# XiangLi2022/CM-TTS

Measured on AMD Instinct MI355X. Metric: mel-frames/s (text->mel hot path, consistency sampling T=4), higher is better.
Workload: dtype f32

## Files before the change

cm-tts_amd/csrc/denoiser_persist.hip:

```cpp
#include <hip/hip_runtime.h>
#include <type_traits>
#include "gate.h"
#include "mfma_lane.h"
#include "persist_args.h"
#include "persist_tail.h"
#include "wino43.h"

typedef float f32x2 __attribute__((ext_vector_type(2)));

#ifndef WINO_ABL
#define WINO_ABL 0
#endif
#ifndef WINO_L2PF
#define WINO_L2PF 0
#endif
#ifndef WINO_THREAD
#define WINO_THREAD 1
#endif
#ifndef WINO43_RING
#define WINO43_RING 3
#endif
#ifndef WINO_RING
#define WINO_RING 3
#endif

namespace {

constexpr int C = 256;
constexpr int NW = 8;
constexpr int MT = 2;
constexpr int RING = 6;
constexpr int FN = 64;
constexpr int NT = FN / 32;
constexpr int U_LD = FN + 4;
constexpr int ROWV = 4 * 32;
constexpr int IDX_LDS_BYTES = (FN + 2) * 2 * 4 + NW * 64 * 4 + NW * 4 + NW * ROWV * 4;
static_assert(((FN + 2) * 2 * 4 + NW * 64 * 4 + NW * 4) % 16 == 0, "row vectors are read 16 bytes at a time");
constexpr unsigned SPIN_LIMIT = 1u << 20;


template <bool DBG, bool RAGGED, bool FACT = false, int WINO = 0>
__global__ __launch_bounds__(64 * NW, 2) void denoiser_persist_kernel(const PersistArgs a) {
    extern __shared__ __attribute__((aligned(16))) float smem[];
    const int tid = threadIdx.x, lane = tid & 63, w = tid >> 6;
    int tile_, b_, T_, Tc_, gi = 0;
    if (RAGGED) {
        const unsigned d = a.desc[blockIdx.x];
        gi = d & 7;
        b_ = (d >> 3) & 1023;
        tile_ = (d >> 13) & 127;
        T_ = a.grp[gi].T;
        Tc_ = min(T_, (int)((d >> 20) & 255) * FN);
    } else {
        tile_ = blockIdx.x; b_ = blockIdx.y; T_ = a.T; Tc_ = a.T;
    }
    const int tile = tile_, b = b_;
    const int t0 = tile * FN;
    const int T = T_;
    const int Tc = Tc_;
    const int l31 = lane & 31, khalf = lane >> 5;
    const float* x0_b = (RAGGED ? a.grp[gi].x0 : a.x0) + (long)b * C * T;
    const float* cp_b = (RAGGED ? a.grp[gi].cp + (long)b * a.grp[gi].cp_bstride : a.cp + (long)b * a.cp_bstride);
    const float* dp_b = (RAGGED ? a.grp[gi].dp : a.dp) + (long)b * a.vec_stride;
    const float* dv_b = (RAGGED ? a.grp[gi].d : a.d) + (long)b * a.vec_stride;
    unsigned long long* halo_g = RAGGED ? a.grp[gi].halo : a.halo;
    const int B_g = RAGGED ? a.grp[gi].B : a.B, tiles_g = RAGGED ? a.grp[gi].tiles : a.tiles;
    const int mrow0 = w * 32;
    const float *p1_b = nullptr, *p1t_b = nullptr;
    const long long *m2p_b = nullptr, *pix_b = nullptr;
    int ldp = 0, Lph = 0;
    if (FACT) {
        p1_b = (RAGGED ? a.grp[gi].p1 : a.p1);
        ldp = RAGGED ? a.grp[gi].ldp : a.ldp;
        Lph = RAGGED ? a.grp[gi].Lph : a.Lph;
        p1_b += (long)b * a.NL * C * ldp;
        p1t_b = (RAGGED ? a.grp[gi].p1t : a.p1t) + (long)b * a.NL * C * ldp;
        m2p_b = (RAGGED ? a.grp[gi].mel2ph : a.mel2ph) + (long)b * T;
        pix_b = (RAGGED ? a.grp[gi].pidx : a.pidx) + (long)b * T;
    }
    auto frame_idx = [&](int t_c, int& ph, int& ix) {
        const long long p = m2p_b[t_c], q = pix_b[t_c];
        ph = (int)(p > Lph ? Lph : p);
        ix = q < 0 ? 0 : (q >= a.ld2 ? a.ld2 - 1 : (int)q);
    };
    auto cp_fact = [&](int row, int ph, int ix) -> float {
        const float av = p1_b[(long)row * ldp + (ph > 0 ? ph - 1 : 0)];
        const float qv = a.p2[(long)row * a.ld2 + ix];
        return (ph > 0 ? av : 0.f) + qv;
    };

    auto uidx = [](int f) { return WINO == 1 ? ((f & 1) ? (f + 1) >> 1 : 33 + (f >> 1)) : f + 1; };
    constexpr int PST_TILE = NW * 8 * 64 * 4;
    float* pst_b = nullptr;
    if (WINO) pst_b = (RAGGED ? a.grp[gi].xst : a.xst) + ((long)b * (RAGGED ? a.grp[gi].tiles : a.tiles) + tile) * PST_TILE;

    {
        const float* xin = x0_b;
        const int t = t0 + lane;
        const int t_c = min(t, T - 1);
        int ph0 = 0, ix0 = 0;
        if (FACT) frame_idx(t_c, ph0, ix0);
        constexpr int ROWS_PER_WAVE = C / NW;
#pragma unroll 1
        for (int i = 0; i < ROWS_PER_WAVE; i += 8) {
            float xv[8], cv[8], dq[8];
#pragma unroll
            for (int q = 0; q < 8; ++q) {
                const int m = w * ROWS_PER_WAVE + i + q;
                xv[q] = xin[(unsigned)(m * T + t_c)];
                cv[q] = FACT ? cp_fact(m, ph0, ix0) : cp_b[(unsigned)(m * T + t_c)];
                dq[q] = dp_b[m];
            }
#pragma unroll
            for (int q = 0; q < 8; ++q) {
                const int m = w * ROWS_PER_WAVE + i + q;
                const float uv = cv[q] + (xv[q] + dq[q]);
                smem[m * U_LD + uidx(lane)] = t < Tc ? uv : 0.f;
            }
        }
        if (tid < 2 * C) {
            const int m = tid & (C - 1);
            const bool right = tid >= C;
            const int th = right ? t0 + FN : t0 - 1;
            const int thc = min(max(th, 0), T - 1);
            float cph0;
            if (FACT) { int ph, ix; frame_idx(thc, ph, ix); cph0 = cp_fact(m, ph, ix); }
            else cph0 = cp_b[(unsigned)(m * T + thc)];
            const float uh = cph0 + (xin[(unsigned)(m * T + thc)] + dp_b[m]);
            smem[m * U_LD + uidx(right ? FN : -1)] = (th >= 0 && th < Tc) ? uh : 0.f;
        }
    }
    int* idx_lds = reinterpret_cast<int*>(smem + 2 * C * U_LD);
    int* zflag = idx_lds + (FN + 2) * 2 + NW * 64;
    if (tid < NW) zflag[tid] = 0;
    float* rowv = reinterpret_cast<float*>(zflag + NW) + w * ROWV;
    constexpr bool ROWV_LDS = WINO != 0;
    if (FACT && tid < FN + 2) {
        int ph, ix;
        frame_idx(min(max(t0 - 1 + tid, 0), T - 1), ph, ix);
        idx_lds[2 * tid] = ph;
        idx_lds[2 * tid + 1] = ix;
    }
    f32x16 st[MT][NT];
    {
        const float* xin = x0_b;
#pragma unroll
        for (int i = 0; i < MT; ++i)
#pragma unroll
            for (int j = 0; j < NT; ++j) {
                const int t_c = min(t0 + j * 32 + l31, T - 1);
#pragma unroll
                for (int r = 0; r < 16; ++r)
                    st[i][j][r] = (i == 0 && !WINO) ? ldg(xin, (unsigned)((mrow0 + acc_row(r, lane)) * T + t_c)) : 0.f;
            }
    }

    f32x16 acc[MT][NT];
    auto load_a = [&](f32x4 (&dst)[MT], const float* wfrag, int group) {
#pragma unroll
        for (int i = 0; i < MT; ++i)
            dst[i] = *reinterpret_cast<const f32x4*>(wfrag + ((long)group * (2 * C / 32) + w * MT + i) * 256 + lane * 4);
    };
    auto load_ao = [&](f32x4 (&dst)[MT], const float* wfrag, int group) {
#pragma unroll
        for (int i = 0; i < MT; ++i)
            dst[i] = *reinterpret_cast<const f32x4*>(wfrag + ((long)group * (2 * C / 32) + i * NW + w) * 256 + lane * 4);
    };
    const f32x16 zero16 = {0.f, 0.f, 0.f, 0.f, 0.f, 0.f, 0.f, 0.f, 0.f, 0.f, 0.f, 0.f, 0.f, 0.f, 0.f, 0.f};
    auto mma_group = [&](auto first, const f32x4 (&af)[MT], const float (&bv)[4][NT], auto i0) {
        constexpr bool FIRST = decltype(first)::value;
        constexpr int I0 = decltype(i0)::value;
#pragma unroll
        for (int kk = 0; kk < 4; ++kk)
#pragma unroll
            for (int i = I0; i < MT; ++i)
#pragma unroll
                for (int j = 0; j < NT; ++j)
                    acc[i][j] = __builtin_amdgcn_mfma_f32_32x32x2f32(af[i][kk], bv[kk][j], FIRST && kk == 0 ? zero16 : acc[i][j], 0, 0, 0);
    };
    using first_t = std::integral_constant<bool, true>;
    using later_t = std::integral_constant<bool, false>;

    const int bid_dbg = blockIdx.x + gridDim.x * blockIdx.y;
#ifdef PUB_STAMP
    constexpr bool PUBS = true;
#else
    constexpr bool PUBS = false;
#endif
    constexpr int DBG_SLOTS = 9;
    auto stamp = [&](int l, int slot) {
        if (DBG && a.dbg && lane == 0) {
            long long* d = a.dbg + ((long)bid_dbg * NW + w) * DBG_SLOTS;
            if (l == a.NL / 2 && !(PUBS && slot < 6)) d[slot] = (long long)__builtin_readcyclecounter();
            if (l == a.NL / 2 + 1 && slot == 0) d[8] = (long long)__builtin_readcyclecounter();
        }
    };
    auto pstamp = [&](int l, int slot) {
        if (DBG && PUBS && a.dbg && l == a.NL / 2 && lane == 0) {
            asm volatile("s_waitcnt lgkmcnt(0)" ::: "memory");
            a.dbg[((long)bid_dbg * NW + w) * DBG_SLOTS + slot] = (long long)__builtin_readcyclecounter();
        }
    };
    bool gave_up = false;
    for (int l = 0; l < a.NL; ++l) {
        float* u_lds = smem;
        float* z_lds = smem + C * U_LD;
        const bool more = l + 1 < a.NL;
        constexpr int NGB = (C / 8) * 3;
        constexpr int NGC = C / 8;
        auto kgrp = [&](int it, int& g8, int& tap) {
            it = min(it, NGB - 1);
            const int q = it / 6, rr = it - q * 6;
            tap = rr >> 1;
            g8 = 2 * q + (rr & 1);
        };
        f32x4 A[RING][MT];
        constexpr int WR = WINO_RING, NH = C / 4;
        f32x4 Aw[WINO == 1 ? WR : 1][MT][2];
        constexpr int WR4 = WINO43_RING, NS4 = C / 4;
        f32x4 A4[WINO == 2 ? WR4 : 1][6];
        auto load_a4 = [&](f32x4 (&dst)[6], const float* wfrag, int ks) {
            const __amdgpu_buffer_rsrc_t rs = __builtin_amdgcn_make_buffer_rsrc(const_cast<float*>(wfrag), 0, (NS4 + 4) * (NW * 6 * 64 * 16), 0x00020000);
            const int voff = (w * 6 * 64 + lane) * 16;
#pragma unroll
            for (int p = 0; p < 6; ++p)
                dst[p] = __builtin_bit_cast(f32x4, __builtin_amdgcn_raw_buffer_load_b128(rs, voff + p * 1024, ks * (NW * 6 * 64 * 16), 0));
        };
        auto load_aw = [&](f32x4 (&dst)[MT][2], const float* wfrag, int hg) {
            const char* base = reinterpret_cast<const char*>(wfrag) + (size_t)hg * ((2 * C / 32) * 2 * 64 * 16);
#pragma unroll
            for (int i = 0; i < MT; ++i)
#pragma unroll
                for (int ps = 0; ps < 2; ++ps)
                    dst[i][ps] = *reinterpret_cast<const f32x4*>(base + (size_t)((unsigned)((((w * MT + i) * 2 + ps) * 64 + lane) * 16)));
        };
        if (WINO == 2) {
#pragma unroll
            for (int s = 0; s < WR4 - 1; ++s) load_a4(A4[s], a.W3f[l], s);
        } else if (WINO == 1) {
#pragma unroll
            for (int s = 0; s < WR - 1; ++s) load_aw(Aw[s], a.W3f[l], s);
        } else {
            int g8, tap;
#pragma unroll
            for (int s = 0; s < RING - 1; ++s) {
                kgrp(s, g8, tap);
                load_a(A[s], a.W3f[l], tap * (C / 8) + g8);
            }
        }
        stamp(l, 0);
        __syncthreads();
        stamp(l, 1);
        if (!FACT && more && tid < 2 * C) {
            const float* cpn = cp_b + (long)(l + 1) * C * T;
            const int tl = opaque(tid);
            const float warm = cpn[(unsigned)((tl >> 1) * T + min(t0 + (tl & 1) * 32, T - 1))];
            asm volatile("" ::"v"(warm));
        }

        f32x16 accw[WINO == 1 ? MT : 1][WINO == 1 ? 4 : 1];
        f32x4 acc4[WINO == 2 ? 4 : 1][WINO == 2 ? 6 : 1];
        if constexpr (WINO == 2) {
#pragma unroll
            for (int i = 0; i < 4; ++i)
#pragma unroll
                for (int p = 0; p < 6; ++p)
#pragma unroll
                    for (int r = 0; r < 4; ++r) acc4[i][p][r] = 0.f;
            const float* W3f = a.W3f[l];
            float V4[6];
            f32x4 Da;
            float2 Db;
            auto load_d4 = [&](int ks) {
                const float* rr = u_lds + (4 * ks + (lane >> 4)) * U_LD + 4 * (lane & 15);
                Da = *reinterpret_cast<const f32x4*>(rr);
                Db = *reinterpret_cast<const float2*>(rr + 4);
            };
            auto transform4 = [&]() { wino43::transform(Da, Db, V4); };
            load_d4(0);
#pragma unroll 1
            for (int s0 = 0; s0 < NS4; s0 += WR4) {
#pragma unroll
                for (int s = 0; s < WR4; ++s) {
                    const int ks = s0 + s;
                    transform4();
                    __builtin_amdgcn_sched_barrier(0);
                    load_a4(A4[(s + WR4 - 1) % WR4], W3f, ks + WR4 - 1);
                    load_d4(ks + 1);
                    if (ks < NS4) {
#pragma unroll
                        for (int p = 0; p < 6; ++p)
#pragma unroll
                            for (int i = 0; i < 4; ++i)
                                acc4[i][p] = __builtin_amdgcn_mfma_f32_16x16x4f32(A4[s][p][i], V4[p], acc4[i][p], 0, 0, 0);
                    }
                    __builtin_amdgcn_sched_barrier(0);
                }
            }
        } else if constexpr (WINO == 1) {
#pragma unroll
            for (int i = 0; i < MT; ++i)
#pragma unroll
                for (int tr = 0; tr < 4; ++tr)
#pragma unroll
                    for (int r = 0; r < 16; ++r) accw[i][tr][r] = 0.f;
            const float* W3f = a.W3f[l];
            float Vb[2][4], Dn[2][4];
            auto load_d = [&](int hg) {
                const float* bs = u_lds + (4 * hg + khalf) * U_LD + l31;
#pragma unroll
                for (int kk = 0; kk < 2; ++kk) {
                    const float* rr = bs + 2 * kk * U_LD;
                    Dn[kk][0] = rr[0]; Dn[kk][2] = rr[1]; Dn[kk][1] = rr[33]; Dn[kk][3] = rr[34];
                }
            };
            auto transform = [&]() {
#pragma unroll
                for (int kk = 0; kk < 2; ++kk) {
                    Vb[kk][0] = Dn[kk][0] - Dn[kk][2];
                    Vb[kk][1] = Dn[kk][1] + Dn[kk][2];
                    Vb[kk][2] = Dn[kk][2] - Dn[kk][1];
                    Vb[kk][3] = Dn[kk][1] - Dn[kk][3];
                }
            };
            load_d(0);
#if WINO_ABL & 2
            transform();
#endif
#pragma unroll 1
            for (int h0 = 0; h0 < NH; h0 += WR) {
#pragma unroll
                for (int s = 0; s < WR; ++s) {
                    const int hg = h0 + s;
#if !(WINO_ABL & 2)
                    transform();
                    __builtin_amdgcn_sched_barrier(0);
#endif
#if !(WINO_ABL & 1)
                    load_aw(Aw[(s + WR - 1) % WR], W3f, hg + WR - 1);
#endif
#if !(WINO_ABL & 2)
                    load_d(hg + 1);
#endif
                    if (hg < NH) {
#pragma unroll
                        for (int kk = 0; kk < 2; ++kk)
#pragma unroll
                            for (int tr = 0; tr < 4; ++tr)
#pragma unroll
                                for (int i = 0; i < MT; ++i)
                                    accw[i][tr] = __builtin_amdgcn_mfma_f32_32x32x2f32(Aw[s][i][tr >> 1][(tr & 1) * 2 + kk], Vb[kk][tr], accw[i][tr], 0, 0, 0);
                    }
#if WINO_THREAD
#pragma unroll
                    for (int q = 0; q < 4; ++q) {
                        __builtin_amdgcn_sched_group_barrier(0x008, 2, 0);
                        __builtin_amdgcn_sched_group_barrier(0x020, 1, 0);
                    }
#pragma unroll
                    for (int q = 0; q < 4; ++q) {
                        __builtin_amdgcn_sched_group_barrier(0x008, 2, 0);
                        __builtin_amdgcn_sched_group_barrier(0x100, 1, 0);
                    }
#endif
                    __builtin_amdgcn_sched_barrier(0);
                }
            }
        } else {
            static_assert(RING == 6, "a ring round is one chunk of six k-groups");
            const __amdgpu_buffer_rsrc_t w3rs = __builtin_amdgcn_make_buffer_rsrc(const_cast<float*>(a.W3f[l]), 0, 3 * (C / 8) * (2 * C / 32) * 1024, 0x00020000);
            const int wvo3 = (w * MT * 64 + lane) * 16;
            auto load_a3 = [&](f32x4 (&dst)[MT], int q, int n) {
                const int qq = q + n / 6, ss = n % 6;
                const int group = (ss >> 1) * (C / 8) + 2 * qq + (ss & 1);
#pragma unroll
                for (int i = 0; i < MT; ++i)
                    dst[i] = __builtin_bit_cast(f32x4, __builtin_amdgcn_raw_buffer_load_b128(w3rs, wvo3 + i * 1024, group * ((2 * C / 32) * 1024), 0));
            };
            float Bv[2][4][NT];
            const float* ub0 = u_lds + khalf * U_LD + l31;
            auto load_b3 = [&](float (&dst)[4][NT], const float* ub, int n) {
                const int ro = (n / 6) * 16 + (n & 1) * 8, col = (n % 6) >> 1;
#pragma unroll
                for (int kk = 0; kk < 4; ++kk)
#pragma unroll
                    for (int j = 0; j < NT; ++j) dst[kk][j] = ub[(ro + 2 * kk) * U_LD + col + j * 32];
            };
            load_b3(Bv[0], ub0, 0);
            auto ring_round = [&](int q, auto first) {
                const float* ub = ub0 + q * 16 * U_LD;
#pragma unroll
                for (int s = 0; s < RING; ++s) {
                    load_a3(A[(s + RING - 1) % RING], q, s + RING - 1);
                    load_b3(Bv[(s + 1) & 1], ub, s + 1);
                    __builtin_amdgcn_sched_barrier(0);
                    if (decltype(first)::value && s == 0) mma_group(first_t{}, A[s], Bv[s & 1], std::integral_constant<int, 0>{});
                    else mma_group(later_t{}, A[s], Bv[s & 1], std::integral_constant<int, 0>{});
                    __builtin_amdgcn_sched_barrier(0);
                }
            };
            ring_round(0, first_t{});
#pragma unroll 1
            for (int q = 1; q < C / 16; ++q) ring_round(q, later_t{});
        }
// ... 221 lines not shown
                }
#pragma unroll
            for (int j = 0; j < NT; ++j)
#pragma unroll
                for (int r = 0; r < 16; ++r) asm volatile("" : "+v"(st[1][j][r]));
        }
        if (!more) break;
        stamp(l, 6);
        pstamp(l, 0);
        __builtin_amdgcn_sched_barrier(0);
        const float* dpn = dp_b + (long)(l + 1) * C;
        const unsigned tag = (unsigned)l + 1;
        unsigned long long* hbase = halo_g + ((((long)(l & 1) * B_g + b) * tiles_g) * 2) * C;
        {
            const int ln = opaque(lane), c31 = ln & 31;
            float* edge = reinterpret_cast<float*>(smem + 2 * C * U_LD) + (FN + 2) * 2 + w * 64;
            if (c31 == 0) {
#pragma unroll
                for (int r = 0; r < 16; ++r) edge[acc_row(r, ln)] = st[0][0][r];
            }
            if (c31 == 31) {
#pragma unroll
                for (int r = 0; r < 16; ++r) edge[32 + acc_row(r, ln)] = st[0][NT - 1][r];
            }
            store_granule(hbase + ((long)tile * 2 + (ln >> 5)) * C + mrow0 + (ln & 31), tag, edge[ln]);
        }
        const int hside = opaque(lane) >> 5, hm = mrow0 + (opaque(lane) & 31);
        const int hth = hside ? t0 + FN : t0 - 1;
        const bool hinside = hth >= 0 && hth < Tc;
        const unsigned long long* hg = hbase + ((long)(hinside ? (hside ? tile + 1 : tile - 1) : tile) * 2 + (hside ? 0 : 1)) * C + hm;
        float hcp = 0.f;
        int hph = 0, hix = 0;
        {
            const int thc = min(max(hth, 0), T - 1);
            if (FACT) { hph = idx_lds[2 * (hside ? FN + 1 : 0)]; hix = idx_lds[2 * (hside ? FN + 1 : 0) + 1]; }
            else hcp = (cp_b + (long)(l + 1) * C * T)[(unsigned)(hm * T + thc)];
        }
        const float hdp = ldg(dpn, (unsigned)hm);
        unsigned long long hv = __hip_atomic_load((gu64*)hg, __ATOMIC_RELAXED, __HIP_MEMORY_SCOPE_AGENT);
        pstamp(l, 1);
        {
            const float* cpn = cp_b + (long)(l + 1) * C * T;
            const int ln = opaque(lane), c31 = ln & 31;
            f32x16 cpc[NT];
            float dpr[16];
            if constexpr (FACT) {
                const float* p1l = p1_b + (long)(l + 1) * C * ldp;
                const float* p2l = a.p2 + (long)(l + 1) * C * a.ld2;
                const float* p1tl = p1t_b + (long)(l + 1) * ldp * C;
                const float* p2tl = a.p2t + (long)(l + 1) * a.ld2 * C;
                int phj[NT], ixj[NT];
#pragma unroll
                for (int j = 0; j < NT; ++j) { phj[j] = idx_lds[2 * (1 + j * 32 + c31)]; ixj[j] = idx_lds[2 * (1 + j * 32 + c31) + 1]; }
                const __amdgpu_buffer_rsrc_t r1t = __builtin_amdgcn_make_buffer_rsrc(const_cast<float*>(p1tl), 0, ldp * C * 4, 0x00020000);
                const __amdgpu_buffer_rsrc_t r2t = __builtin_amdgcn_make_buffer_rsrc(const_cast<float*>(p2tl), 0, a.ld2 * C * 4, 0x00020000);
                const __amdgpu_buffer_rsrc_t r1 = __builtin_amdgcn_make_buffer_rsrc(const_cast<float*>(p1l), 0, C * ldp * 4, 0x00020000);
                const __amdgpu_buffer_rsrc_t r2 = __builtin_amdgcn_make_buffer_rsrc(const_cast<float*>(p2l), 0, C * a.ld2 * 4, 0x00020000);
                f32x4 g1[NT][4], g2[NT][4];
                const float h1 = __builtin_bit_cast(float, __builtin_amdgcn_raw_buffer_load_b32(r1, (int)((unsigned)(hm * ldp + (hph > 0 ? hph - 1 : 0)) * 4u), 0, 0));
                const float h2 = __builtin_bit_cast(float, __builtin_amdgcn_raw_buffer_load_b32(r2, (int)((unsigned)(hm * a.ld2 + hix) * 4u), 0, 0));
#pragma unroll
                for (int j = 0; j < NT; ++j) {
                    const int o1 = (int)((unsigned)((phj[j] > 0 ? phj[j] - 1 : 0) * C + mrow0 + 4 * (ln >> 5)) * 4u);
                    const int o2 = (int)((unsigned)(ixj[j] * C + mrow0 + 4 * (ln >> 5)) * 4u);
#pragma unroll
                    for (int q = 0; q < 4; ++q) {
                        g1[j][q] = __builtin_bit_cast(f32x4, __builtin_amdgcn_raw_buffer_load_b128(r1t, o1 + q * 32, 0, 0));
                        g2[j][q] = __builtin_bit_cast(f32x4, __builtin_amdgcn_raw_buffer_load_b128(r2t, o2 + q * 32, 0, 0));
                    }
                }
                if constexpr (!ROWV_LDS) {
                    const __amdgpu_buffer_rsrc_t rd = __builtin_amdgcn_make_buffer_rsrc(const_cast<float*>(dpn), 0, C * 4, 0x00020000);
                    const int od = (int)((unsigned)(mrow0 + 4 * (ln >> 5)) * 4u);
#pragma unroll
                    for (int r = 0; r < 16; ++r)
                        dpr[r] = __builtin_bit_cast(float, __builtin_amdgcn_raw_buffer_load_b32(rd, od + ((r & 3) + 8 * (r >> 2)) * 4, 0, 0));
                }
                pstamp(l, 2);
                hcp = (hph > 0 ? h1 : 0.f) + h2;
#pragma unroll
                for (int j = 0; j < NT; ++j)
#pragma unroll
                    for (int q = 0; q < 4; ++q) {
#pragma unroll
                        for (int e = 0; e < 4; ++e) cpc[j][4 * q + e] = (phj[j] > 0 ? g1[j][q][e] : 0.f) + g2[j][q][e];
                    }
            } else {
#pragma unroll
                for (int j = 0; j < NT; ++j) {
                    const int t_c = min(t0 + j * 32 + c31, T - 1);
#pragma unroll
                    for (int r = 0; r < 16; ++r) cpc[j][r] = ldg(cpn, (unsigned)((mrow0 + acc_row(r, ln)) * T + t_c));
                }
                if constexpr (!ROWV_LDS) {
#pragma unroll
                    for (int r = 0; r < 16; ++r) dpr[r] = ldg(dpn, (unsigned)(mrow0 + acc_row(r, ln)));
                }
            }
            if constexpr (ROWV_LDS) {
#pragma unroll
                for (int q = 0; q < 4; ++q) {
                    const f32x4 dq = *reinterpret_cast<const f32x4*>(rowv + 96 + 4 * (ln >> 5) + 8 * q);
#pragma unroll
                    for (int e = 0; e < 4; ++e) dpr[4 * q + e] = dq[e];
                }
            }
#pragma unroll
            for (int j = 0; j < NT; ++j) {
                const int t = t0 + j * 32 + c31;
#pragma unroll
                for (int r = 0; r < 16; ++r) {
                    const int m = mrow0 + acc_row(r, ln);
                    const float uv = cpc[j][r] + (st[0][j][r] + dpr[r]);
                    u_lds[m * U_LD + uidx(j * 32 + c31)] = t < Tc ? uv : 0.f;
                }
            }
        }
        pstamp(l, 3);
        {
            if (!gave_up) {
                unsigned spins = 0;
                while (!__all(!hinside || (unsigned)(hv >> 32) == tag)) {
                    if (++spins > SPIN_LIMIT) {
                        if (lane == 0 && a.tmo) *(volatile unsigned*)a.tmo = 1u;
                        gave_up = true;
                        break;
                    }
                    __builtin_amdgcn_s_sleep(4);
                    hv = __hip_atomic_load((gu64*)hg, __ATOMIC_RELAXED, __HIP_MEMORY_SCOPE_AGENT);
                }
            }
            const float xh = gave_up ? __builtin_nanf("") : (hinside ? __uint_as_float((unsigned)hv) : 0.f);
            const float uh = hcp + (xh + hdp);
            u_lds[hm * U_LD + uidx(hside ? FN : -1)] = hinside ? uh : 0.f;
        }
        pstamp(l, 4);
        if constexpr (WINO) {
            f32x4* px = reinterpret_cast<f32x4*>(pst_b) + (w * 8) * 64 + opaque(lane);
#pragma unroll
            for (int j = 0; j < NT; ++j)
#pragma unroll
                for (int q = 0; q < 4; ++q) {
                    f32x4 vx;
#pragma unroll
                    for (int e = 0; e < 4; ++e) vx[e] = st[0][j][4 * q + e];
                    px[(j * 4 + q) * 64] = vx;
                }
        }
        pstamp(l, 5);
        stamp(l, 7);
    }

    if (a.tail) {
        persist_tail::run(a, smem, smem + C * U_LD, st[1], w, lane, b, t0, T, RAGGED ? a.grp[gi].xold : a.xold,
                          RAGGED ? a.grp[gi].noise : a.noise, RAGGED ? a.grp[gi].out : a.out, Tc, !RAGGED);
    } else {
        float* skip = (RAGGED ? a.grp[gi].skip : a.skip) + (long)b * C * T;
#pragma unroll
        for (int j = 0; j < NT; ++j) {
            const int t = t0 + j * 32 + l31;
#pragma unroll
            for (int r = 0; r < 16; ++r)
                if (t < Tc) skip[(unsigned)((mrow0 + acc_row(r, lane)) * T + t)] = st[1][j][r];
        }
    }
}

long long* g_pdbg = nullptr;
int g_coop = -1;
int g_process_group = 0;
constexpr int N_VARIANTS = 24;
int g_validated_wg[N_VARIANTS] = {};

}

extern "C" int cmtts_persist_set_cooperative(int on) { const int p = g_coop; if (on >= -1 && on <= 1) g_coop = on; return p; }
extern "C" int cmtts_persist_note_process_group(int on) { const int p = g_process_group; if (on == 0 || on == 1) g_process_group = on; return p; }
extern "C" int cmtts_persist_cooperative(int variant, int gx, int gy) {
    if (g_coop >= 0) return g_coop;
    if (!g_process_group) return 0;
    const long wg = (long)gx * (gy > 0 ? gy : 1);
    if (variant < 0 || variant >= N_VARIANTS) return 1;
    return wg > g_validated_wg[variant] ? 1 : 0;
}
extern "C" void cmtts_persist_validated(int variant, int gx, int gy) {
    const long wg = (long)gx * (gy > 0 ? gy : 1);
    if (variant >= 0 && variant < N_VARIANTS && wg > g_validated_wg[variant]) g_validated_wg[variant] = (int)wg;
}

extern "C" void cmtts_persist_set_debug(long long* dbg) { g_pdbg = dbg; }
extern "C" long long* cmtts_persist_get_debug(void) { return g_pdbg; }

extern "C" int cmtts_persist_chunks(int B, int T, int max_blocks) {
    if (B < 1 || T < 1 || max_blocks < 1) return 0;
    const int tiles = (T + FN - 1) / FN;
    if (tiles > max_blocks) return 0;
    const int per_launch = max_blocks / tiles;
    return (B + per_launch - 1) / per_launch;
}

extern "C" int cmtts_persist_plan(int B, int T, int NL, int max_blocks, int force) {
    const int tiles = (T + FN - 1) / FN;
    if (B < 1 || T < 1 || max_blocks < 1 || NL < 1 || NL > PERSIST_MAX_LAYERS || tiles > max_blocks || (long)C * T >= (1L << 30)) return 0;
    if (!force && (long)tiles * B * 2 <= (long)max_blocks) return 0;
    const int per_launch = max_blocks / tiles;
    const int nchunks = (B + per_launch - 1) / per_launch;
    const int bc = (B + nchunks - 1) / nchunks;
    return tiles * (bc < B ? bc : B);
}

extern "C" size_t cmtts_persist_state_floats(int B, int T) {
    const long tiles = (T + FN - 1) / FN;
    return (size_t)B * tiles * (NW * 8 * 64 * 4);
}

extern "C" size_t cmtts_persist_halo_bytes(int B, int T) {
    const long tiles = (T + FN - 1) / FN;
    return (size_t)2 * B * tiles * 2 * C * sizeof(unsigned long long);
}

extern "C" int cmtts_launch_denoiser_persist(const PersistArgs* a_in, int max_blocks, int force, void* stream_) {
    PersistArgs a = *a_in;
    hipStream_t stream = (hipStream_t)stream_;
    if (a.B < 1 || a.T < 1 || max_blocks < 1) return -2;
    const int tiles = (a.T + FN - 1) / FN;
    if (a.NL < 1 || a.NL > PERSIST_MAX_LAYERS || tiles > max_blocks || (long)C * a.T >= (1L << 30)) return -2;
    if (!force && (long)tiles * a.B * 2 <= (long)max_blocks) return -2;
    a.tiles = tiles;
    a.dbg = g_pdbg;
    if ((a.wino == 1 || a.wino == 3) && !a.xst) return -2;
    const int wsel = a.wino == 3 ? 2 : a.wino ? 1 : 0;
    if (a.wino == 2) return -2;
    const int threads = 64 * NW;
#define KFN(D, R, F, W) reinterpret_cast<const void*>(denoiser_persist_kernel<D, R, F, W>)
    static const void* const kfns[2][2][3] = {
        {{KFN(false, false, false, 0), KFN(false, false, false, 1), KFN(false, false, false, 2)}, {KFN(false, false, true, 0), KFN(false, false, true, 1), KFN(false, false, true, 2)}},
        {{KFN(true, false, false, 0), KFN(true, false, false, 1), KFN(true, false, false, 2)}, {KFN(true, false, true, 0), KFN(true, false, true, 1), KFN(true, false, true, 2)}}};
    static bool attr_set = false;
    const size_t lds = (size_t)2 * C * U_LD * sizeof(float) + IDX_LDS_BYTES;
    if (!attr_set) {
        for (int d = 0; d < 2; ++d)
            for (int f = 0; f < 2; ++f) {
                for (int wn = 0; wn < 3; ++wn)
                    if (hipFuncSetAttribute(kfns[d][f][wn], hipFuncAttributeMaxDynamicSharedMemorySize, (int)lds) != hipSuccess) return -3;
            }
        attr_set = true;
    }
    if (a.fact && (!a.p1 || !a.p2 || !a.mel2ph || !a.pidx || a.ldp < 1 || a.ld2 < 1)) return -2;
    if (a.fact && (!a.p1t || !a.p2t)) return -2;
    if (!a.halo_zeroed && hipMemsetAsync(a.halo, 0, cmtts_persist_halo_bytes(a.B, a.T), stream) != hipSuccess) return -3;
    const int B = a.B;
    const int per_launch = max_blocks / tiles;
    const int nchunks = (B + per_launch - 1) / per_launch;
    const int bc = (B + nchunks - 1) / nchunks;
    for (int b0 = 0; b0 < B; b0 += bc) {
        PersistArgs c = a;
        const int nb = B - b0 < bc ? B - b0 : bc;
        c.x0 = a.x0 + (long)b0 * C * a.T;
        c.cp = a.cp + (long)b0 * a.cp_bstride;
        c.dp = a.dp + (long)b0 * a.vec_stride;
        c.d = a.d + (long)b0 * a.vec_stride;
        c.skip = a.skip + (long)b0 * C * a.T;
        if (a.xst) c.xst = a.xst + (long)b0 * tiles * (NW * 8 * 64 * 4);
        c.halo = a.halo + (long)b0 * tiles * 2 * C;
        if (a.fact) {
            c.p1 = a.p1 + (long)b0 * a.NL * C * a.ldp;
            if (a.p1t) c.p1t = a.p1t + (long)b0 * a.NL * C * a.ldp;
            c.mel2ph = a.mel2ph + (long)b0 * a.T;
            c.pidx = a.pidx + (long)b0 * a.T;
        }
        if (a.tail) {
            const long off = (long)b0 * a.T * a.n_mels;
            c.xold = a.xold ? a.xold + off : nullptr;
            c.noise = a.noise ? a.noise + off : nullptr;
            c.out = a.out + off;
            if (a.post_rows) c.post_rows = a.post_rows + b0;
            if (a.out_final) c.out_final = a.out_final + off;
        }
        const void* kfn = kfns[a.dbg ? 1 : 0][a.fact ? 1 : 0][wsel];
        void* params[] = {(void*)&c};
        const int variant = wsel * 2 + (a.fact ? 1 : 0);
        if (!a.dbg && cmtts_persist_cooperative(variant, tiles, nb)) {
            if (hipLaunchCooperativeKernel(kfn, dim3(tiles, nb), dim3(threads), params, (unsigned)lds, stream) != hipSuccess) return -3;
            cmtts_persist_validated(variant, tiles, nb);
        } else if (hipLaunchKernel(kfn, dim3(tiles, nb), dim3(threads), params, lds, stream) != hipSuccess) return -3;
        if (hipGetLastError() != hipSuccess) return -3;
    }
    return 0;
}

extern "C" int cmtts_launch_denoiser_persist_ragged(const PersistArgs* a_in, void* stream_) {
    const PersistArgs& a = *a_in;
    hipStream_t stream = (hipStream_t)stream_;
    if (a.NL < 1 || a.NL > PERSIST_MAX_LAYERS || a.n_groups < 1 || a.n_groups > PERSIST_MAX_GROUPS || a.n_wg < 1 || a.n_wg > PERSIST_MAX_WG)
        return -2;
    for (int g = 0; g < a.n_groups; ++g)
        if ((long)C * a.grp[g].T >= (1L << 30) || a.grp[g].tiles > 127 || a.grp[g].B > 1023) return -2;
    static const void* const kfns[2][3] = {{KFN(false, true, false, 0), KFN(false, true, false, 1), KFN(false, true, false, 2)},
                                           {KFN(false, true, true, 0), KFN(false, true, true, 1), KFN(false, true, true, 2)}};
    static bool attr_set = false;
    const size_t lds = (size_t)2 * C * U_LD * sizeof(float) + IDX_LDS_BYTES;
    if (!attr_set) {
        for (int f = 0; f < 2; ++f) {
            for (int wn = 0; wn < 3; ++wn)
                if (hipFuncSetAttribute(kfns[f][wn], hipFuncAttributeMaxDynamicSharedMemorySize, (int)lds) != hipSuccess) return -3;
        }
        attr_set = true;
    }
// ... 24 lines not shown
```

cm-tts_amd/csrc/persist_tail.h:

```cpp
#pragma once
#include <hip/hip_runtime.h>
#include "mfma_lane.h"
#include "persist_args.h"

namespace persist_tail {

constexpr int PT_C = 256, PT_NT = 2, PT_LD = 68, PT_RING = 6;

template <int TPW = 1>
__device__ __forceinline__ void run(const PersistArgs& a, float* u_lds, float* z_lds, const f32x16* skip, int w, int lane,
                                    int b, int t0, int T, const float* xold, const float* noise, float* out, int Tc, bool rows = true) {
    constexpr int C = PT_C, NT = PT_NT, U_LD = PT_LD, RING = PT_RING;
    const int l31 = lane & 31, khalf = lane >> 5;
    const bool table = rows && a.post_rows != nullptr;
    unsigned row_w[4] = {0u, 0u, 0u, 0u};
    if (table) {
        const unsigned* pr = reinterpret_cast<const unsigned*>(a.post_rows + b);
#pragma unroll
        for (int i = 0; i < 4; ++i) row_w[i] = pr[i];
    }
    {
        const int ln = opaque(lane), c31 = ln & 31;
#pragma unroll
        for (int i = 0; i < TPW; ++i)
#pragma unroll
            for (int j = 0; j < NT; ++j)
#pragma unroll
                for (int r = 0; r < 16; ++r)
                    u_lds[((w * TPW + i) * 32 + acc_row(r, ln)) * U_LD + j * 32 + c31] = skip[i * NT + j][r] / a.skip_div;
    }
    __syncthreads();
    float c_out = a.c_out, c_skip = a.c_skip, nstd = a.nstd;
    if (table) {
        c_out = __uint_as_float(__builtin_amdgcn_readfirstlane(row_w[0]));
        c_skip = __uint_as_float(__builtin_amdgcn_readfirstlane(row_w[1]));
        nstd = __uint_as_float(__builtin_amdgcn_readfirstlane(row_w[2]));
        const unsigned flags = __builtin_amdgcn_readfirstlane(row_w[3]);
        if (!(flags & POSTROW_RENOISE)) noise = nullptr;
        if (flags & POSTROW_FINAL) out = a.out_final;
    }
    constexpr int NGC = C / 8;
    auto load_bt = [&](float (&dst)[4][NT], const float* src, int g) {
        const float* bs = src + (g * 8 + khalf) * U_LD + l31;
#pragma unroll
        for (int kk = 0; kk < 4; ++kk)
#pragma unroll
            for (int j = 0; j < NT; ++j) dst[kk][j] = bs[2 * kk * U_LD + j * 32];
    };
    f32x16 h[NT];
    auto gemm_tile = [&](const float* wfrag, int mtiles, int mt, const float* src) {
#pragma unroll
        for (int j = 0; j < NT; ++j)
#pragma unroll
            for (int r = 0; r < 16; ++r) h[j][r] = 0.f;
        f32x4 Af[RING];
        float Bt[2][4][NT];
#pragma unroll
        for (int s = 0; s < RING - 1; ++s)
            Af[s] = *reinterpret_cast<const f32x4*>(wfrag + (((long)min(s, NGC - 1) * mtiles + mt) * 64 + lane) * 4);
        load_bt(Bt[0], src, 0);
#pragma unroll 1
        for (int it = 0; it < NGC; it += RING) {
#pragma unroll
            for (int s = 0; s < RING; ++s) {
                Af[(s + RING - 1) % RING] =
                    *reinterpret_cast<const f32x4*>(wfrag + (((long)min(it + s + RING - 1, NGC - 1) * mtiles + mt) * 64 + lane) * 4);
                load_bt(Bt[(s + 1) & 1], src, min(it + s + 1, NGC - 1));
                __builtin_amdgcn_sched_barrier(0);
                if (it + s < NGC) {
#pragma unroll
                    for (int kk = 0; kk < 4; ++kk)
#pragma unroll
                        for (int j = 0; j < NT; ++j)
                            h[j] = __builtin_amdgcn_mfma_f32_32x32x2f32(Af[s][kk], Bt[s & 1][kk][j], h[j], 0, 0, 0);
                }
                __builtin_amdgcn_sched_barrier(0);
            }
        }
    };
#pragma unroll
    for (int i = 0; i < TPW; ++i) {
        const int mrow0 = (w * TPW + i) * 32;
        gemm_tile(a.Wsf, C / 32, w * TPW + i, u_lds);
        const int ln = opaque(lane), c31 = ln & 31;
#pragma unroll
        for (int r = 0; r < 16; ++r) {
            const int m = mrow0 + acc_row(r, ln);
            const float bi = ldg(a.bs, (unsigned)m);
#pragma unroll
            for (int j = 0; j < NT; ++j) {
                float v = h[j][r] + bi;
                v *= 1.0f;
                v = v > 0.f ? v : 0.f;
                z_lds[m * U_LD + j * 32 + c31] = v;
            }
        }
    }
    __syncthreads();
    const int otiles = (a.n_mels + 31) / 32;
    if (w < otiles) {
        const int mrow0 = w * 32;
        gemm_tile(a.Wpf, otiles, w, z_lds);
        const int ln = opaque(lane), c31 = ln & 31;
        const int M = a.n_mels;
        float bi[16];
#pragma unroll
        for (int r = 0; r < 16; ++r) bi[r] = ldg(a.bp, (unsigned)min(mrow0 + acc_row(r, ln), M - 1));
        bool bad = false;
#pragma unroll
        for (int j = 0; j < NT; ++j) {
            const int t = t0 + j * 32 + c31;
            const long ob = ((long)b * T + min(t, T - 1)) * M;
            float xo[16], nz[16];
            if (xold) {
#pragma unroll
                for (int r = 0; r < 16; ++r) xo[r] = xold[ob + min(mrow0 + acc_row(r, ln), M - 1)];
            }
            if (noise) {
#pragma unroll
                for (int r = 0; r < 16; ++r) nz[r] = noise[ob + min(mrow0 + acc_row(r, ln), M - 1)];
            }
#pragma unroll
            for (int r = 0; r < 16; ++r) {
                const int m = mrow0 + acc_row(r, ln);
                const bool ok = m < M && t < Tc;
                const float F = h[j][r] + (m < M ? bi[r] : 0.f);
                float v = c_out * F;
                if (xold) v = __builtin_fmaf(c_skip, xo[r], v);
                if (noise) v = __builtin_fmaf(nz[r] * nstd, 0.85f, v);
                if (ok) out[ob + m] = v;
                bad |= ok && !(fabsf(v) <= 3.402823466e38f);
            }
        }
        if (bad && a.tmo && *(volatile unsigned*)a.tmo == 0u) *(volatile unsigned*)a.tmo = 2u;
    }
}

}
```

Before: 2.008 million.

## Vectorize factored prologue loads and split tail output GEMM across more waves

The prologue now reads the factored conditioning from transposed p1t/p2t tables using 128-bit buffer loads, issues all row and halo loads up front, and writes the idx_lds entries in the same pass. This replaces the old strided scalar loads and the separate index pass. In the tail, the skip-GEMM bias loads and the first weight-ring prefetch are hoisted ahead of the barrier. The output projection is split per column tile so twice as many waves share it, and its xold/noise loads are issued before the barrier to overlap the sync. Debug cycle stamps are added, and the new code relies on p1t/p2t transposed layouts being present.

New measurement: 2.008 million. Within noise of the previous version (-0.0%).

```diff
diff --git a/cm-tts_amd/csrc/denoiser_persist.hip b/cm-tts_amd/csrc/denoiser_persist.hip
--- a/cm-tts_amd/csrc/denoiser_persist.hip
+++ b/cm-tts_amd/csrc/denoiser_persist.hip
@@ -78,69 +78,85 @@
         m2p_b = (RAGGED ? a.grp[gi].mel2ph : a.mel2ph) + (long)b * T;
         pix_b = (RAGGED ? a.grp[gi].pidx : a.pidx) + (long)b * T;
     }
-    auto frame_idx = [&](int t_c, int& ph, int& ix) {
-        const long long p = m2p_b[t_c], q = pix_b[t_c];
-        ph = (int)(p > Lph ? Lph : p);
-        ix = q < 0 ? 0 : (q >= a.ld2 ? a.ld2 - 1 : (int)q);
-    };
-    auto cp_fact = [&](int row, int ph, int ix) -> float {
-        const float av = p1_b[(long)row * ldp + (ph > 0 ? ph - 1 : 0)];
-        const float qv = a.p2[(long)row * a.ld2 + ix];
-        return (ph > 0 ? av : 0.f) + qv;
-    };
 
     auto uidx = [](int f) { return WINO == 1 ? ((f & 1) ? (f + 1) >> 1 : 33 + (f >> 1)) : f + 1; };
     constexpr int PST_TILE = NW * 8 * 64 * 4;
     float* pst_b = nullptr;
     if (WINO) pst_b = (RAGGED ? a.grp[gi].xst : a.xst) + ((long)b * (RAGGED ? a.grp[gi].tiles : a.tiles) + tile) * PST_TILE;
 
+    constexpr int DBG_SLOTS = 17;
+    long long* const dbg_w = (DBG && a.dbg) ? a.dbg + ((long)(blockIdx.x + gridDim.x * blockIdx.y) * NW + w) * DBG_SLOTS : nullptr;
+    auto estamp = [&](int slot) {
+        if (DBG && dbg_w && lane == 0) dbg_w[slot] = (long long)__builtin_readcyclecounter();
+    };
+    estamp(9);
+    int* idx_lds = reinterpret_cast<int*>(smem + 2 * C * U_LD);
     {
         const float* xin = x0_b;
         const int t = t0 + lane;
         const int t_c = min(t, T - 1);
-        int ph0 = 0, ix0 = 0;
-        if (FACT) frame_idx(t_c, ph0, ix0);
         constexpr int ROWS_PER_WAVE = C / NW;
-#pragma unroll 1
-        for (int i = 0; i < ROWS_PER_WAVE; i += 8) {
-            float xv[8], cv[8], dq[8];
-#pragma unroll
-            for (int q = 0; q < 8; ++q) {
-                const int m = w * ROWS_PER_WAVE + i + q;
-                xv[q] = xin[(unsigned)(m * T + t_c)];
-                cv[q] = FACT ? cp_fact(m, ph0, ix0) : cp_b[(unsigned)(m * T + t_c)];
-                dq[q] = dp_b[m];
-            }
-#pragma unroll
-            for (int q = 0; q < 8; ++q) {
-                const int m = w * ROWS_PER_WAVE + i + q;
-                const float uv = cv[q] + (xv[q] + dq[q]);
-                smem[m * U_LD + uidx(lane)] = t < Tc ? uv : 0.f;
-            }
-        }
-        if (tid < 2 * C) {
-            const int m = tid & (C - 1);
-            const bool right = tid >= C;
-            const int th = right ? t0 + FN : t0 - 1;
-            const int thc = min(max(th, 0), T - 1);
-            float cph0;
-            if (FACT) { int ph, ix; frame_idx(thc, ph, ix); cph0 = cp_fact(m, ph, ix); }
-            else cph0 = cp_b[(unsigned)(m * T + thc)];
-            const float uh = cph0 + (xin[(unsigned)(m * T + thc)] + dp_b[m]);
-            smem[m * U_LD + uidx(right ? FN : -1)] = (th >= 0 && th < Tc) ? uh : 0.f;
-        }
+        static_assert(ROWS_PER_WAVE % 4 == 0 && 2 * C == 64 * NW, "16-byte runs of a wave's rows; one halo entry per thread");
+        const int hm0 = tid & (C - 1);
+        const bool right = tid >= C;
+        const int th = right ? t0 + FN : t0 - 1;
+        const int thc = min(max(th, 0), T - 1);
+        long long fp = 0, fq = 0, hp = 0, hq = 0;
+        if (FACT) { fp = m2p_b[t_c]; fq = pix_b[t_c]; hp = m2p_b[thc]; hq = pix_b[thc]; }
+        float xv[ROWS_PER_WAVE], cv[ROWS_PER_WAVE], dq[ROWS_PER_WAVE];
+#pragma unroll
+        for (int q = 0; q < ROWS_PER_WAVE; ++q) {
+            const int m = w * ROWS_PER_WAVE + q;
+            xv[q] = xin[(unsigned)(m * T + t_c)];
+            if (!FACT) cv[q] = cp_b[(unsigned)(m * T + t_c)];
+            dq[q] = dp_b[m];
+        }
+        const float xh = xin[(unsigned)(hm0 * T + thc)];
+        const float dh = dp_b[hm0];
+        float ch = 0.f;
+        if constexpr (FACT) {
+            auto clamp_idx = [&](long long p, long long q, int& ph, int& ix) {
+                ph = (int)(p > Lph ? Lph : p);
+                ix = q < 0 ? 0 : (q >= a.ld2 ? a.ld2 - 1 : (int)q);
+            };
+            int ph0, ix0, hph0, hix0;
+            clamp_idx(fp, fq, ph0, ix0);
+            clamp_idx(hp, hq, hph0, hix0);
+            const __amdgpu_buffer_rsrc_t r1t = __builtin_amdgcn_make_buffer_rsrc(const_cast<float*>(p1t_b), 0, ldp * C * 4, 0x00020000);
+            const __amdgpu_buffer_rsrc_t r2t = __builtin_amdgcn_make_buffer_rsrc(const_cast<float*>(a.p2t), 0, a.ld2 * C * 4, 0x00020000);
+            const int o1 = (int)((unsigned)((ph0 > 0 ? ph0 - 1 : 0) * C + w * ROWS_PER_WAVE) * 4u);
+            const int o2 = (int)((unsigned)(ix0 * C + w * ROWS_PER_WAVE) * 4u);
+            f32x4 g1[ROWS_PER_WAVE / 4], g2[ROWS_PER_WAVE / 4];
+#pragma unroll
+            for (int q = 0; q < ROWS_PER_WAVE / 4; ++q) {
+                g1[q] = __builtin_bit_cast(f32x4, __builtin_amdgcn_raw_buffer_load_b128(r1t, o1 + q * 16, 0, 0));
+                g2[q] = __builtin_bit_cast(f32x4, __builtin_amdgcn_raw_buffer_load_b128(r2t, o2 + q * 16, 0, 0));
+            }
+            const float h1 = __builtin_bit_cast(float, __builtin_amdgcn_raw_buffer_load_b32(r1t, (int)((unsigned)((hph0 > 0 ? hph0 - 1 : 0) * C + hm0) * 4u), 0, 0));
+            const float h2 = __builtin_bit_cast(float, __builtin_amdgcn_raw_buffer_load_b32(r2t, (int)((unsigned)(hix0 * C + hm0) * 4u), 0, 0));
+            if (w == 0) { idx_lds[2 * (1 + lane)] = ph0; idx_lds[2 * (1 + lane) + 1] = ix0; }
+            if (lane == 0 && (tid == 0 || tid == C)) { idx_lds[2 * (right ? FN + 1 : 0)] = hph0; idx_lds[2 * (right ? FN + 1 : 0) + 1] = hix0; }
+#pragma unroll
+            for (int q = 0; q < ROWS_PER_WAVE / 4; ++q)
+#pragma unroll
+                for (int e = 0; e < 4; ++e) cv[4 * q + e] = (ph0 > 0 ? g1[q][e] : 0.f) + g2[q][e];
+            ch = (hph0 > 0 ? h1 : 0.f) + h2;
+        } else {
+            ch = cp_b[(unsigned)(hm0 * T + thc)];
+        }
+#pragma unroll
+        for (int q = 0; q < ROWS_PER_WAVE; ++q) {
+            const int m = w * ROWS_PER_WAVE + q;
+            const float uv = cv[q] + (xv[q] + dq[q]);
+            smem[m * U_LD + uidx(lane)] = t < Tc ? uv : 0.f;
+        }
+        const float uh = ch + (xh + dh);
+        smem[hm0 * U_LD + uidx(right ? FN : -1)] = (th >= 0 && th < Tc) ? uh : 0.f;
     }
-    int* idx_lds = reinterpret_cast<int*>(smem + 2 * C * U_LD);
     int* zflag = idx_lds + (FN + 2) * 2 + NW * 64;
     if (tid < NW) zflag[tid] = 0;
     float* rowv = reinterpret_cast<float*>(zflag + NW) + w * ROWV;
     constexpr bool ROWV_LDS = WINO != 0;
-    if (FACT && tid < FN + 2) {
-        int ph, ix;
-        frame_idx(min(max(t0 - 1 + tid, 0), T - 1), ph, ix);
-        idx_lds[2 * tid] = ph;
-        idx_lds[2 * tid + 1] = ix;
-    }
     f32x16 st[MT][NT];
     {
         const float* xin = x0_b;
@@ -187,7 +203,6 @@
 #else
     constexpr bool PUBS = false;
 #endif
-    constexpr int DBG_SLOTS = 9;
     auto stamp = [&](int l, int slot) {
         if (DBG && a.dbg && lane == 0) {
             long long* d = a.dbg + ((long)bid_dbg * NW + w) * DBG_SLOTS;
@@ -249,7 +264,9 @@
             }
         }
         stamp(l, 0);
+        if (DBG && l == 0) estamp(10);
         __syncthreads();
+        if (DBG && l == 0) estamp(11);
         stamp(l, 1);
         if (!FACT && more && tid < 2 * C) {
             const float* cpn = cp_b + (long)(l + 1) * C * T;
@@ -777,8 +794,9 @@
     }
 
     if (a.tail) {
-        persist_tail::run(a, smem, smem + C * U_LD, st[1], w, lane, b, t0, T, RAGGED ? a.grp[gi].xold : a.xold,
-                          RAGGED ? a.grp[gi].noise : a.noise, RAGGED ? a.grp[gi].out : a.out, Tc, !RAGGED);
+        estamp(12);
+        persist_tail::run<1, DBG>(a, smem, smem + C * U_LD, st[1], w, lane, b, t0, T, RAGGED ? a.grp[gi].xold : a.xold,
+                                  RAGGED ? a.grp[gi].noise : a.noise, RAGGED ? a.grp[gi].out : a.out, Tc, !RAGGED, dbg_w);
     } else {
         float* skip = (RAGGED ? a.grp[gi].skip : a.skip) + (long)b * C * T;
 #pragma unroll
diff --git a/cm-tts_amd/csrc/persist_tail.h b/cm-tts_amd/csrc/persist_tail.h
--- a/cm-tts_amd/csrc/persist_tail.h
+++ b/cm-tts_amd/csrc/persist_tail.h
@@ -1,5 +1,6 @@
 #pragma once
 #include <hip/hip_runtime.h>
+#include <type_traits>
 #include "mfma_lane.h"
 #include "persist_args.h"
 
@@ -7,11 +8,16 @@
 
 constexpr int PT_C = 256, PT_NT = 2, PT_LD = 68, PT_RING = 6;
 
-template <int TPW = 1>
+template <int TPW = 1, bool DBG = false>
 __device__ __forceinline__ void run(const PersistArgs& a, float* u_lds, float* z_lds, const f32x16* skip, int w, int lane,
-                                    int b, int t0, int T, const float* xold, const float* noise, float* out, int Tc, bool rows = true) {
+                                    int b, int t0, int T, const float* xold, const float* noise, float* out, int Tc, bool rows = true,
+                                    long long* dbgw = nullptr) {
     constexpr int C = PT_C, NT = PT_NT, U_LD = PT_LD, RING = PT_RING;
+    constexpr bool SPLIT = TPW == 1;
     const int l31 = lane & 31, khalf = lane >> 5;
+    auto stamp = [&](int slot) {
+        if (DBG && dbgw && lane == 0) dbgw[slot] = (long long)__builtin_readcyclecounter();
+    };
     const bool table = rows && a.post_rows != nullptr;
     unsigned row_w[4] = {0u, 0u, 0u, 0u};
     if (table) {
@@ -19,6 +25,24 @@
 #pragma unroll
         for (int i = 0; i < 4; ++i) row_w[i] = pr[i];
     }
+    constexpr int NGC = C / 8;
+    auto load_af = [&](const float* wfrag, int mtiles, int mt, int g) -> f32x4 {
+        return *reinterpret_cast<const f32x4*>(wfrag + (((long)min(g, NGC - 1) * mtiles + mt) * 64 + lane) * 4);
+    };
+    auto ring_head = [&](f32x4 (&Af)[RING], const float* wfrag, int mtiles, int mt) {
+#pragma unroll
+        for (int s = 0; s < RING - 1; ++s) Af[s] = load_af(wfrag, mtiles, mt, s);
+    };
+    float bsr[TPW][16];
+    {
+        const int ln = opaque(lane);
+#pragma unroll
+        for (int i = 0; i < TPW; ++i)
+#pragma unroll
+            for (int r = 0; r < 16; ++r) bsr[i][r] = ldg(a.bs, (unsigned)((w * TPW + i) * 32 + acc_row(r, ln)));
+    }
+    f32x4 Af[RING];
+    ring_head(Af, a.Wsf, C / 32, w * TPW);
     {
         const int ln = opaque(lane), c31 = ln & 31;
 #pragma unroll
@@ -30,6 +54,7 @@
                     u_lds[((w * TPW + i) * 32 + acc_row(r, ln)) * U_LD + j * 32 + c31] = skip[i * NT + j][r] / a.skip_div;
     }
     __syncthreads();
+    stamp(13);
     float c_out = a.c_out, c_skip = a.c_skip, nstd = a.nstd;
     if (table) {
         c_out = __uint_as_float(__builtin_amdgcn_readfirstlane(row_w[0]));
@@ -39,54 +64,52 @@
         if (!(flags & POSTROW_RENOISE)) noise = nullptr;
         if (flags & POSTROW_FINAL) out = a.out_final;
     }
-    constexpr int NGC = C / 8;
-    auto load_bt = [&](float (&dst)[4][NT], const float* src, int g) {
-        const float* bs = src + (g * 8 + khalf) * U_LD + l31;
+    auto gemm_tile = [&](auto ntl, f32x16 (&h)[NT], f32x4 (&Af)[RING], const float* wfrag, int mtiles, int mt, const float* src) {
+        constexpr int NTL = decltype(ntl)::value;
+        auto load_bt = [&](float (&dst)[4][NTL], int g) {
+            const float* bs = src + (g * 8 + khalf) * U_LD + l31;
 #pragma unroll
-        for (int kk = 0; kk < 4; ++kk)
+            for (int kk = 0; kk < 4; ++kk)
 #pragma unroll
-            for (int j = 0; j < NT; ++j) dst[kk][j] = bs[2 * kk * U_LD + j * 32];
-    };
-    f32x16 h[NT];
-    auto gemm_tile = [&](const float* wfrag, int mtiles, int mt, const float* src) {
+                for (int j = 0; j < NTL; ++j) dst[kk][j] = bs[2 * kk * U_LD + j * 32];
+        };
 #pragma unroll
-        for (int j = 0; j < NT; ++j)
+        for (int j = 0; j < NTL; ++j)
 #pragma unroll
             for (int r = 0; r < 16; ++r) h[j][r] = 0.f;
-        f32x4 Af[RING];
-        float Bt[2][4][NT];
-#pragma unroll
-        for (int s = 0; s < RING - 1; ++s)
-            Af[s] = *reinterpret_cast<const f32x4*>(wfrag + (((long)min(s, NGC - 1) * mtiles + mt) * 64 + lane) * 4);
-        load_bt(Bt[0], src, 0);
+        float Bt[2][4][NTL];
+        load_bt(Bt[0], 0);
 #pragma unroll 1
         for (int it = 0; it < NGC; it += RING) {
 #pragma unroll
             for (int s = 0; s < RING; ++s) {
-                Af[(s + RING - 1) % RING] =
-                    *reinterpret_cast<const f32x4*>(wfrag + (((long)min(it + s + RING - 1, NGC - 1) * mtiles + mt) * 64 + lane) * 4);
-                load_bt(Bt[(s + 1) & 1], src, min(it + s + 1, NGC - 1));
+                Af[(s + RING - 1) % RING] = load_af(wfrag, mtiles, mt, it + s + RING - 1);
+                load_bt(Bt[(s + 1) & 1], min(it + s + 1, NGC - 1));
                 __builtin_amdgcn_sched_barrier(0);
                 if (it + s < NGC) {
 #pragma unroll
                     for (int kk = 0; kk < 4; ++kk)
 #pragma unroll
-                        for (int j = 0; j < NT; ++j)
+                        for (int j = 0; j < NTL; ++j)
                             h[j] = __builtin_amdgcn_mfma_f32_32x32x2f32(Af[s][kk], Bt[s & 1][kk][j], h[j], 0, 0, 0);
                 }
                 __builtin_amdgcn_sched_barrier(0);
             }
         }
     };
+    using ntl_all = std::integral_constant<int, NT>;
+    using ntl_one = std::integral_constant<int, 1>;
+    f32x16 h[NT];
 #pragma unroll
     for (int i = 0; i < TPW; ++i) {
         const int mrow0 = (w * TPW + i) * 32;
-        gemm_tile(a.Wsf, C / 32, w * TPW + i, u_lds);
+        if (i > 0) ring_head(Af, a.Wsf, C / 32, w * TPW + i);
+        gemm_tile(ntl_all{}, h, Af, a.Wsf, C / 32, w * TPW + i, u_lds);
         const int ln = opaque(lane), c31 = ln & 31;
 #pragma unroll
         for (int r = 0; r < 16; ++r) {
             const int m = mrow0 + acc_row(r, ln);
-            const float bi = ldg(a.bs, (unsigned)m);
+            const float bi = bsr[i][r];
 #pragma unroll
             for (int j = 0; j < NT; ++j) {
                 float v = h[j][r] + bi;
@@ -96,44 +119,59 @@
             }
         }
     }
-    __syncthreads();
     const int otiles = (a.n_mels + 31) / 32;
-    if (w < otiles) {
-        const int mrow0 = w * 32;
-        gemm_tile(a.Wpf, otiles, w, z_lds);
+    constexpr int ONT = SPLIT ? 1 : NT;
+    const bool owork = w < (SPLIT ? otiles * NT : otiles);
+    const int omt = SPLIT ? w % otiles : w, oj0 = SPLIT ? w / otiles : 0;
+    const int M = a.n_mels;
+    float bi[16], xo[ONT][16], nz[ONT][16];
+    if (owork) {
+        ring_head(Af, a.Wpf, otiles, omt);
         const int ln = opaque(lane), c31 = ln & 31;
-        const int M = a.n_mels;
-        float bi[16];
 #pragma unroll
-        for (int r = 0; r < 16; ++r) bi[r] = ldg(a.bp, (unsigned)min(mrow0 + acc_row(r, ln), M - 1));
-        bool bad = false;
+        for (int r = 0; r < 16; ++r) bi[r] = ldg(a.bp, (unsigned)min(omt * 32 + acc_row(r, ln), M - 1));
 #pragma unroll
-        for (int j = 0; j < NT; ++j) {
-            const int t = t0 + j * 32 + c31;
+        for (int jj = 0; jj < ONT; ++jj) {
+            const int t = t0 + (oj0 + jj) * 32 + c31;
             const long ob = ((long)b * T + min(t, T - 1)) * M;
-            float xo[16], nz[16];
             if (xold) {
 #pragma unroll
-                for (int r = 0; r < 16; ++r) xo[r] = xold[ob + min(mrow0 + acc_row(r, ln), M - 1)];
+                for (int r = 0; r < 16; ++r) xo[jj][r] = xold[ob + min(omt * 32 + acc_row(r, ln), M - 1)];
             }
             if (noise) {
 #pragma unroll
-                for (int r = 0; r < 16; ++r) nz[r] = noise[ob + min(mrow0 + acc_row(r, ln), M - 1)];
+                for (int r = 0; r < 16; ++r) nz[jj][r] = noise[ob + min(omt * 32 + acc_row(r, ln), M - 1)];
             }
+        }
+    }
+    stamp(14);
+    __syncthreads();
+    stamp(15);
+    if (owork) {
+        const int mrow0 = omt * 32;
+        if constexpr (SPLIT) gemm_tile(ntl_one{}, h, Af, a.Wpf, otiles, omt, z_lds + oj0 * 32);
+        else gemm_tile(ntl_all{}, h, Af, a.Wpf, otiles, omt, z_lds);
+        const int ln = opaque(lane), c31 = ln & 31;
+        bool bad = false;
+#pragma unroll
+        for (int jj = 0; jj < ONT; ++jj) {
+            const int t = t0 + (oj0 + jj) * 32 + c31;
+            const long ob = ((long)b * T + min(t, T - 1)) * M;
 #pragma unroll
             for (int r = 0; r < 16; ++r) {
                 const int m = mrow0 + acc_row(r, ln);
                 const bool ok = m < M && t < Tc;
-                const float F = h[j][r] + (m < M ? bi[r] : 0.f);
+                const float F = h[jj][r] + (m < M ? bi[r] : 0.f);
                 float v = c_out * F;
-                if (xold) v = __builtin_fmaf(c_skip, xo[r], v);
-                if (noise) v = __builtin_fmaf(nz[r] * nstd, 0.85f, v);
+                if (xold) v = __builtin_fmaf(c_skip, xo[jj][r], v);
+                if (noise) v = __builtin_fmaf(nz[jj][r] * nstd, 0.85f, v);
                 if (ok) out[ob + m] = v;
                 bad |= ok && !(fabsf(v) <= 3.402823466e38f);
             }
         }
         if (bad && a.tmo && *(volatile unsigned*)a.tmo == 0u) *(volatile unsigned*)a.tmo = 2u;
     }
+    stamp(16);
 }
 
 }
```
